# Rhizomatica/mercury

Measured on AMD Instinct MI355X. Metric: RX frames/s (mode 8, max 50 LDPC iters), higher is better.
Workload: dtype f64

## Files before the change

### include/mercury_gpu.h

```cpp
#ifndef MERCURY_GPU_H
#define MERCURY_GPU_H

#include <stddef.h>
#include <stdint.h>

#ifdef __cplusplus
extern "C" {
#endif

#define MGPU_OK 0
#define MGPU_ERR_ARG 1
#define MGPU_ERR_DEVICE 2
#define MGPU_ERR_TABLES 3
#define MGPU_ERR_UNSUPPORTED 4

#define MGPU_DEC_GBF 0
#define MGPU_DEC_SPA 1
#define MGPU_DEC_MINSUM 2
#define MGPU_DEC_SPA_FAST 3

#define MGPU_EST_ZF 0
#define MGPU_EST_LS 1

typedef struct mgpu_ctx mgpu_ctx;
// ... 6 lines not shown
         ? -1                                                                                                                     \
         : 1000 + (((MGPU_CFG_MOD_INDEX_(M) * 8 + MGPU_CFG_RATE_INDEX_(rate16)) * 8 + ((preamble_nsymb)-1)) * 2 + (estimator)))

typedef struct mgpu_config {
    int cfg;
    int max_iters;
    int decoder;
    int agc;
    int variance_source;
    int device;
    int max_batch;
    float minsum_alpha;
    int mfsk_ctrl_mode;
    int test_puncture_nBits;
} mgpu_config;

typedef struct mgpu_info {
    int cfg, M, bits_per_symbol, K, P, N;
    int Nsymb, Nc, Nfft, Ngi, Nofdm;
    int nData, nBits, nPilots, nVirtual, nReal;
    int bit_blk, tf_blk, preamble_nsymb;
    int estimator, amp_restore, ls_window;
    int Cwidth, Vwidth, E;
    int payload_bytes;
    int payload_stride;
    int frame_samples;
    int mfsk_M, mfsk_nStreams;
    int active_nsymb, active_nbits;
} mgpu_info;

typedef struct mgpu_frame_stats {
    int iterations_done;
    int crc;
    int all_zeros;
    int message_decoded;
    float variance;
    float snr_db;
} mgpu_frame_stats;

typedef struct mgpu_stage_taps {
    double* grid;
    double* H;
    double* eq;
    double* syms;
    float* llr_demod;
    float* llr_ldpc;
    double* variance;
    double* agc_gain;
    long long* cycles;
} mgpu_stage_taps;

int mgpu_create(const mgpu_config* cfg, mgpu_ctx** out);

typedef struct mgpu_explicit_params {
    float pilot_boost;
    int ls_window;
    int seeds_set;
    unsigned pilot_seed, scrambler_seed, preamble_seed;
    int Nc, Nfft, Dx;
    int Dy;
    int Nsymb;
} mgpu_explicit_params;
int mgpu_create_explicit(const mgpu_config* cfg, const mgpu_explicit_params* params, mgpu_ctx** out);
void mgpu_destroy(mgpu_ctx* ctx);
const char* mgpu_last_error(mgpu_ctx* ctx);
int mgpu_get_info(mgpu_ctx* ctx, mgpu_info* info);

void* mgpu_alloc_host(size_t bytes);
void mgpu_free_host(void* p);

typedef struct mgpu_device_props {
    int compute_units, clock_khz, memory_clock_khz, lds_bytes_per_cu, wavefront_size, numa_node;
    unsigned long long hbm_bytes;
    char name[64];
    char gcn_arch[32];
    char pci_bus_id[32];
} mgpu_device_props;
int mgpu_device_props_get(int device, mgpu_device_props* out);
void* mgpu_alloc_host_near(int device, size_t bytes);
int mgpu_host_numa_node_of_pci(const char* pci_bus_id);
int mgpu_host_numa_cpus(int node, int* cpus, int max);

int mgpu_rx_batch(mgpu_ctx* ctx, const double* baseband_c128, int F, uint8_t* payload,
                  mgpu_frame_stats* stats, float* llr_opt);
int mgpu_rx_batch_taps(mgpu_ctx* ctx, const double* baseband_c128, int F, uint8_t* payload,
                       mgpu_frame_stats* stats, const mgpu_stage_taps* taps);
int mgpu_ldpc_batch(mgpu_ctx* ctx, const float* llr, int F, uint8_t* bits, int* iters);
int mgpu_host_select_peak(const double* cand_vals, int ncand, int step, int size, int location_to_return, int nTrials_max, int* delay,
                          double* correlation);
int mgpu_host_fir_taps(int which, double carrier_hz, double* taps, int* ntaps);
int mgpu_host_preamble_carriers(int cfg, double* carriers_c128, int* n_symbols);
int mgpu_host_mode_info(int cfg, int mfsk_ctrl_mode, mgpu_info* info);
int mgpu_host_layout_stats(int cfg, double out[4]);

typedef struct mgpu_libm_report {
    long long evaluated[4], differed[4];
    double first_differing_argument[4];
    int differing;
    char libc_version[32];
} mgpu_libm_report;
int mgpu_host_libm_selfcheck(mgpu_libm_report* out );

int mgpu_ldpc_encode_batch(mgpu_ctx* ctx, const uint8_t* bits, int F, uint8_t* encoded);

int mgpu_rx_batch_dev(mgpu_ctx* ctx, const void* d_baseband_c128, int F, void* d_payload,
                      void* d_stats, void* d_llr_opt, void* stream);
int mgpu_frontend_dev(mgpu_ctx* ctx, const void* d_baseband_c128, int F, void* d_llr, void* d_variance_f,
                      void* stream);
int mgpu_ldpc_batch_dev(mgpu_ctx* ctx, const void* d_llr, int F, void* d_bits_opt, void* d_iters,
                        void* d_payload_opt, void* d_stats_opt, const void* d_variance_f_opt, void* stream);
void* mgpu_device_malloc(mgpu_ctx* ctx, size_t bytes);
void mgpu_device_free(mgpu_ctx* ctx, void* d_ptr);
void* mgpu_context_stream(mgpu_ctx* ctx);
int mgpu_synchronize(mgpu_ctx* ctx, void* stream_or_null);
int mgpu_copy_to_host(mgpu_ctx* ctx, void* dst, const void* d_src, size_t bytes, void* stream_or_null);
int mgpu_copy_to_device(mgpu_ctx* ctx, void* d_dst, const void* src, size_t bytes, void* stream_or_null);
int mgpu_txgen_dev(mgpu_ctx* ctx, uint64_t seed, uint64_t frame0, int F, double noise_amp, int channel,
                   void* d_baseband_c128, void* d_payload_opt, void* stream);

typedef struct mgpu_error_rate {
    double esn0_db;
    long long Frames_total, Error_frames_total, Bits_total, Error_bits_total;
    double BER, FER;
    double avg_iterations;
    long long crc_ok_frames;
} mgpu_error_rate;
int mgpu_baseband_test_esn0(mgpu_ctx* ctx, const double* esn0_db, int npoints, long long frames_per_point, uint64_t seed, uint64_t frame0,
                            int channel, mgpu_error_rate* out);

int mgpu_passband_to_baseband(mgpu_ctx* ctx, const double* passband , int W, int in_size,
                              const double* carrier_hz , int filter, const int* start , int count,
                              int decimation, double* out_c128 );
int mgpu_time_sync_preamble(mgpu_ctx* ctx, const double* baseband_interp_c128 , int W, int size, int step,
                            int location_to_return, int nTrials_max, int* delay , double* correlation );
int mgpu_freq_sync(mgpu_ctx* ctx, const double* baseband_c128 , int W, int stride, double* freq_offset_hz );
int mgpu_time_sync_mfsk(mgpu_ctx* ctx, const double* baseband_interp_c128 , int W, int size, int search_start_symb,
                        int* delay );
int mgpu_detect_ack_pattern(mgpu_ctx* ctx, const double* baseband_interp_c128 , int W, int size, int pattern,
                            double* metric , int* matched );
int mgpu_detect_ack_pattern_from_passband(mgpu_ctx* ctx, const double* passband , int W, int size, double carrier_hz,
                                          int pattern, double* metric , int* matched );
int mgpu_last_sync_kernel_ms(mgpu_ctx* ctx, float* ms);

int mgpu_enable_timing(mgpu_ctx* ctx, int on);
int mgpu_kernel_ms_avg(mgpu_ctx* ctx, float ms[2], int* n_launches);
int mgpu_decoder_hard_frames(mgpu_ctx* ctx, long long* frames);
int mgpu_host_path_last(mgpu_ctx* ctx, int* chunk_frames, int* n_chunks, float* fill_ms, float* drain_ms, float* total_ms);
int mgpu_last_kernel_ms(mgpu_ctx* ctx, float ms[2]);

int mgpu_debug_mfsk_sync(mgpu_ctx* ctx, const double* energy, int W, int nslots, int size, const int* search_start, int variant, int* delay);
int mgpu_debug_p2b_variant(int variant);
int mgpu_debug_span_energy(mgpu_ctx* ctx, const double* bb, int W, int size, const int* wv, const int* off, int n, int len, int variant, double* sum,
                           int* cnt);
int mgpu_debug_spa_math(mgpu_ctx* ctx, const double* in, int n, double* tanh_out, double* atanh_out);
int mgpu_debug_select_peak(mgpu_ctx* ctx, const double* cand_vals, int n, int ncand_max, const int* ncand, const int* size, const int* loc, int step,
                           int nTrials_max, int* delay, double* corr);

int mgpu_debug_occupancy(mgpu_ctx* ctx, int which);

int mgpu_debug_tsync_metric(mgpu_ctx* ctx, const double* baseband_interp, int W, int size, int step, int variant, const int* start, const int* sub_size,
                            double* vals);

int mgpu_debug_glibc_trig(mgpu_ctx* ctx, const double* in, int n, double* atan_out, double* sin_out, double* cos_out);

#ifdef __cplusplus
}
#endif
#endif
```

### mercury_amd/csrc/tables.cpp

```cpp
#include "tables.hpp"
#include "device_tables.h"

#include <algorithm>
#include <complex>
#include <cmath>
#include <cstring>
#include <future>
#include <map>
#include <memory>
#include <mutex>
#include <stdexcept>

namespace mgpu {

void GlibcRandom::reseed(unsigned seed) {
    if (seed == 0) seed = 1;
    st_[0] = static_cast<int32_t>(seed);
    int32_t word = st_[0];
    for (int i = 1; i < 31; ++i) {
        const long hi = word / 127773, lo = word % 127773;
        word = static_cast<int32_t>(16807 * lo - 2836 * hi);
        if (word < 0) word += 2147483647;
        st_[i] = word;
    }
    f_ = 3;
    r_ = 0;
    for (int k = 0; k < 310; ++k) (void)next();
}

int32_t GlibcRandom::next() {
    const uint32_t val = static_cast<uint32_t>(st_[f_]) + static_cast<uint32_t>(st_[r_]);
    st_[f_] = static_cast<int32_t>(val);
    if (++f_ >= 31) { f_ = 0; ++r_; }
    else if (++r_ >= 31) r_ = 0;
    return static_cast<int32_t>(val >> 1);
}

uint16_t crc16_modbus(const uint8_t* bytes, int n) {
    uint16_t crc = 0xffff;
    for (int j = 0; j < n; ++j) {
        crc ^= bytes[j];
        for (int i = 0; i < 8; ++i) crc = (crc & 1) ? static_cast<uint16_t>((crc >> 1) ^ 0xA001) : static_cast<uint16_t>(crc >> 1);
    }
    return crc;
}

namespace {

struct ModeRow { int M, rate16, preamble, estimator; };
constexpr ModeRow kModeTable[17] = {
    {2, 1, 4, 1},  {2, 2, 4, 1},  {2, 3, 4, 1},  {2, 4, 4, 1},  {2, 5, 4, 1},  {2, 6, 4, 1},
    {2, 8, 4, 1},  {4, 5, 4, 1},  {4, 6, 4, 1},  {4, 8, 4, 1},  {8, 6, 3, 1},  {8, 8, 3, 1},
    {4, 14, 3, 1}, {16, 8, 2, 1}, {8, 14, 2, 1}, {16, 14, 2, 0}, {32, 14, 1, 0},
};

constexpr int8_t kQam32[32][2] = {
    {-3, 5}, {-1, 5}, {-3, -5}, {-1, -5}, {-5, 3}, {-5, 1}, {-5, -3}, {-5, -1},
    {-1, 3}, {-1, 1}, {-1, -3}, {-1, -1}, {-3, 3}, {-3, 1}, {-3, -3}, {-3, -1},
    {3, 5},  {1, 5},  {3, -5},  {1, -5},  {5, 3},  {5, 1},  {5, -3},  {5, -1},
    {1, 3},  {1, 1},  {1, -3},  {1, -1},  {3, 3},  {3, 1},  {3, -3},  {3, -1}};

std::vector<Cplx> make_constellation(int M) {
    std::vector<Cplx> c(M);
    switch (M) {
        case 2: c = {{1, 0}, {-1, 0}}; break;
        case 4: c = {{-1, 1}, {-1, -1}, {1, 1}, {1, -1}}; break;
        case 8: {
            const double h = std::sqrt(2.0);
            const double p = (1 * h) / 2.0, n = (-1 * h) / 2.0;
            c = {{n, n}, {-1, 0}, {0, 1}, {n, p}, {0, -1}, {p, n}, {p, p}, {1, 0}};
            break;
        }
        case 16:
            for (int s = 0; s < 16; ++s)
                c[s] = {((s & 8) ? 1.0 : -1.0) * ((s & 4) ? 1.0 : 3.0), ((s & 2) ? -1.0 : 1.0) * ((s & 1) ? 1.0 : 3.0)};
            break;
        case 32:
            for (int s = 0; s < 32; ++s) c[s] = {double(kQam32[s][0]), double(kQam32[s][1])};
            break;
        default: throw std::runtime_error("unsupported constellation size");
    }
    float pnv = 0;
    for (const Cplx& z : c) pnv = static_cast<float>(static_cast<double>(pnv) + (z.re * z.re + z.im * z.im));
    const float mean = pnv / static_cast<float>(M);
    pnv = static_cast<float>(1.0 / std::sqrt(static_cast<double>(mean)));
    for (Cplx& z : c) { z.re *= static_cast<double>(pnv); z.im *= static_cast<double>(pnv); }
    return c;
}

std::vector<uint8_t> make_pilot_lattice(int Nsymb, int Nc, int Dy) {
    const int Dx = 1;
    const int S = Nc > Nsymb ? Nc : Nsymb;
    std::vector<uint8_t> v(size_t(S) * S, 0);
    for (int x = 0, y = 0; x < S && y < S; x += Dx, ++y) {
        for (int j = y; j < S; j += Dy) v[size_t(j) * S + x] = 1;
        for (int j = y; j >= 0; j -= Dy) v[size_t(j) * S + x] = 1;
    }
    int in_last = 0;
    for (int j = 0; j < Nsymb; ++j) in_last += v[size_t(j) * S + Nc - 1];
    if (in_last < 2)
        for (int j = 0; j < S; ++j) v[size_t(j) * S + Nc - 1] = v[size_t(j) * S];
    std::vector<uint8_t> t(size_t(Nsymb) * Nc);
    for (int j = 0; j < Nsymb; ++j)
        for (int i = 0; i < Nc; ++i) t[size_t(j) * Nc + i] = v[size_t(j) * S + i];
    return t;
}

static LdpcGraph load_graph_uncached(int K, const uint8_t* blob, size_t size) {
    auto rd32 = [&](size_t off) { uint32_t x; if (off + 4 > size) throw std::runtime_error("LDPC table blob truncated"); std::memcpy(&x, blob + off, 4); return x; };
    if (size < 12 || std::memcmp(blob, "MLDP", 4) != 0 || rd32(4) != 1) throw std::runtime_error("LDPC table blob: bad magic/version");
    const uint32_t nrates = rd32(8);
    size_t off = 12;
    for (uint32_t r = 0; r < nrates; ++r) {
        const uint32_t k = rd32(off), P = rd32(off + 4), N = rd32(off + 8), E = rd32(off + 12), cw = rd32(off + 16), vw = rd32(off + 20);
        off += 24;
        const size_t need = size_t(P) + 2 * size_t(E) + N + 2 * size_t(E);
        if (off + need > size) throw std::runtime_error("LDPC table blob truncated");
        if (int(k) != K) { off += need; continue; }
        LdpcGraph g;
        if (N != 1600) throw std::runtime_error("LDPC table blob: N must be 1600 (the decoders' LDS layout is fixed to it)");
        g.K = K; g.P = P; g.N = N; g.E = E; g.Cwidth = cw; g.Vwidth = vw;
        const uint8_t* cdeg = blob + off;
        const uint8_t* cflat = cdeg + P;
        const uint8_t* vdeg = cflat + 2 * size_t(E);
        const uint8_t* vflat = vdeg + N;
        g.cptr.resize(P + 1); g.cvar.resize(E); g.vptr.resize(N + 1); g.vedge.resize(E);
        uint32_t e = 0;
        for (uint32_t c = 0; c < P; ++c) {
            g.cptr[c] = e;
            for (uint32_t j = 0; j < cdeg[c]; ++j, ++e) {
                uint16_t v; std::memcpy(&v, cflat + 2 * size_t(e), 2);
                g.cvar[e] = v;
            }
        }
        g.cptr[P] = e;
        uint32_t s = 0;
        for (uint32_t v = 0; v < N; ++v) {
            g.vptr[v] = s;
            for (uint32_t j = 0; j < vdeg[v]; ++j, ++s) {
                uint16_t c; std::memcpy(&c, vflat + 2 * size_t(s), 2);
                uint32_t found = UINT32_MAX;
                for (uint32_t q = g.cptr[c]; q < g.cptr[c] + cdeg[c]; ++q)
                    if (g.cvar[q] == v) { found = q; break; }
                if (found == UINT32_MAX) throw std::runtime_error("LDPC table blob: C/V adjacency mismatch");
                g.vedge[s] = uint16_t(found);
            }
        }
        g.vptr[N] = s;
        if (s != E) throw std::runtime_error("LDPC table blob: edge count mismatch");
        std::vector<uint32_t> order(P);
        for (uint32_t c = 0; c < P; ++c) order[c] = c;
        std::stable_sort(order.begin(), order.end(), [&](uint32_t a, uint32_t b) { return cdeg[a] > cdeg[b]; });
        std::vector<int> fill;
        std::vector<std::vector<uint32_t>> members;
        for (uint32_t c : order) {
            const int d = cdeg[c];
            if (d > 64) throw std::runtime_error("check degree exceeds a wavefront");
            size_t b = 0;
            for (; b < fill.size(); ++b) if (fill[b] + d <= 64) break;
            if (b == fill.size()) { fill.push_back(0); members.emplace_back(); }
            fill[b] += d;
            members[b].push_back(c);
        }
        g.S = int(fill.size()) * 64;
        if (g.S >= 8192) throw std::runtime_error("padded edge count exceeds the 13-bit slot field");
        std::vector<uint32_t> slot_of_edge(E);
        for (size_t b = 0; b < members.size(); ++b) {
            uint32_t p = uint32_t(b) * 64;
            for (uint32_t c : members[b]) {
                const uint32_t d = cdeg[c];
                for (uint32_t j = 0; j < d; ++j, ++p) slot_of_edge[g.cptr[c] + j] = p;
            }
        }
        std::vector<uint32_t> vorder(N);
        for (uint32_t v = 0; v < N; ++v) vorder[v] = v;
        std::stable_sort(vorder.begin(), vorder.end(), [&](uint32_t a, uint32_t b) { return vdeg[a] > vdeg[b]; });
        g.vinfo.assign(size_t(N) * 8, 0u);
        for (uint32_t i = 0; i < N; ++i) {
            const uint32_t v = vorder[i], d = vdeg[v];
            if (d > uint32_t(kSpaMaxVarDegree)) throw std::runtime_error("variable degree exceeds the unrolled update (and the bound the fp64 decoder's hard-frame shortcut is proved with: device_tables.h kSpaMaxVarDegree)");
            if (i >= 1024 && d > 4) g.fp64_limit = "variable degrees exceed the fp64 decoder's register layout (rows from 1024 on: at most 4 edges)";
            g.vinfo[size_t(i) * 8] = v | (d << 11);
            for (uint32_t j = 0; j < d; ++j) {
                const uint32_t slot = slot_of_edge[g.vedge[g.vptr[v] + j]];
                g.vinfo[size_t(i) * 8 + 1 + j / 2] |= slot << (16 * (j & 1));
            }
        }
        {
            std::vector<std::vector<uint32_t>> by_kind(7);
            for (uint32_t c : order) {
                int k = 1;
                while ((1 << k) < int(cdeg[c])) ++k;
                by_kind[k].push_back(c);
            }
            std::vector<uint32_t> kinds;
            std::vector<std::vector<uint32_t>> bin_checks;
            for (int k = 6; k >= 1; --k) {
                const size_t per = size_t(64) >> k;
                for (size_t i = 0; i < by_kind[k].size(); i += per) {
                    kinds.push_back(uint32_t(k));
                    bin_checks.emplace_back(by_kind[k].begin() + i, by_kind[k].begin() + std::min(by_kind[k].size(), i + per));
                }
            }
            const size_t bins = kinds.size(), rounds = (bins + 7) / 8;
            g.Sg = int(bins) * 64;
            if (g.Sg >= 65536) throw std::runtime_error("grouped layout exceeds the 16-bit slot index of the variable records");
            if (rounds > 21) throw std::runtime_error("grouped layout exceeds the 21 rounds whose group sizes fit one 64-bit word per wavefront");
            g.gdesc.assign((rounds + 1) * 512, 0u);
            g.gkind.assign((rounds + 1) * 8, 0u);
            g.gkpack.assign(8, 0ull);
            std::vector<uint32_t> lane_of_edge(E), bin_of_edge(E), group_of_edge(E), gsize_of_edge(E);
            for (size_t b = 0; b < bins; ++b) {
                g.gkind[b] = kinds[b];
                g.gkpack[b & 7] |= uint64_t(kinds[b]) << (3 * (b >> 3));
                const uint32_t gsz = 1u << kinds[b];
                for (size_t q = 0; q < bin_checks[b].size(); ++q) {
                    const uint32_t c = bin_checks[b][q];
                    for (uint32_t j = 0; j < cdeg[c]; ++j) {
                        const uint32_t eo = g.cptr[c] + j;
                        lane_of_edge[eo] = uint32_t(q) * gsz + j;
                        bin_of_edge[eo] = uint32_t(b);
                        group_of_edge[eo] = c;
                        gsize_of_edge[eo] = gsz;
                    }
                }
            }
            std::vector<uint32_t> vorder_g = vorder, row_of(N);
            {
                std::vector<std::vector<uint32_t>> halves_of_var(N);
                for (uint32_t c = 0; c < P; ++c)
                    for (uint32_t j = 0; j < cdeg[c]; ++j) {
                        const uint32_t eo = g.cptr[c] + j, h = bin_of_edge[eo] * 2 + (lane_of_edge[eo] >= 32 ? 1u : 0u);
                        auto& hv = halves_of_var[g.cvar[eo]];
                        if (std::find(hv.begin(), hv.end(), h) == hv.end()) hv.push_back(h);
                    }
                std::vector<int> cnt(bins * 2 * 32, 0);
                auto bump = [&](uint32_t v, uint32_t bank, int d) { long long delta = 0; for (uint32_t h : halves_of_var[v]) { int& x = cnt[size_t(h) * 32 + bank]; delta += d > 0 ? 2 * x + 1 : 1 - 2 * x; x += d; } return delta; };
                for (uint32_t i = 0; i < N; ++i) bump(vorder_g[i], i & 31, +1);
                uint32_t lcg = 12345u;
                auto coin = [&] { lcg = lcg * 1664525u + 1013904223u; return (lcg >> 16) & 1u; };
                auto try_swap = [&](uint32_t ia, uint32_t ib) {
                    const uint32_t va = vorder_g[ia], vb = vorder_g[ib];
                    if ((ia & 31) == (ib & 31)) return false;
                    const long long d = bump(va, ia & 31, -1) + bump(vb, ib & 31, -1) + bump(va, ib & 31, +1) + bump(vb, ia & 31, +1);
                    if (d < 0 || (d == 0 && coin())) { std::swap(vorder_g[ia], vorder_g[ib]); return d < 0; }
                    bump(va, ib & 31, -1); bump(vb, ia & 31, -1); bump(va, ia & 31, +1); bump(vb, ib & 31, +1);
                    return false;
                };
                for (int sweep = 0, idle = 0; sweep < 200 && idle < 6; ++sweep) {
                    bool improved = false;
                    for (uint32_t ia = 0; ia < N; ++ia) {
                        const uint32_t lo = ia & ~31u, hi = std::min<uint32_t>(lo + 32, N);
                        for (uint32_t ib = ia + 1; ib < hi; ++ib) improved |= try_swap(ia, ib);
                        for (uint32_t ib = hi; ib < N && ib / 512 == ia / 512 && vdeg[vorder_g[ib]] == vdeg[vorder_g[ia]]; ++ib) improved |= try_swap(ia, ib);
                    }
                    idle = improved ? 0 : idle + 1;
                }
                for (uint32_t i = 0; i < N; ++i) row_of[vorder_g[i]] = i;
            }
            {
                std::vector<uint32_t> access_of_edge(E);
                for (uint32_t v = 0; v < N; ++v)
                    for (uint32_t j = 0; j < vdeg[v]; ++j) access_of_edge[g.vedge[g.vptr[v] + j]] = (row_of[v] / 32) * 9 + j;
                std::vector<int> cnt(size_t((N + 31) / 32) * 9 * 32, 0);
                auto at = [&](uint32_t e, uint32_t lane) -> int& { return cnt[size_t(access_of_edge[e]) * 32 + (lane & 31)]; };
                for (uint32_t e2 = 0; e2 < E; ++e2) ++at(e2, lane_of_edge[e2]);
                uint32_t lcg = 54321u;
                auto coin = [&] { lcg = lcg * 1664525u + 1013904223u; return (lcg >> 16) & 1u; };
                for (int sweep = 0, idle = 0; sweep < 200 && idle < 6; ++sweep) {
                    bool improved = false;
                    for (uint32_t c = 0; c < P; ++c) {
                        const uint32_t e0 = g.cptr[c], d = cdeg[c];
                        if (d == 0) continue;
                        const uint32_t gsz = gsize_of_edge[e0], gbase = lane_of_edge[e0] - (lane_of_edge[e0] % gsz);
                        std::vector<int> edge_at(gsz, -1);
                        for (uint32_t j = 0; j < d; ++j) edge_at[lane_of_edge[e0 + j] - gbase] = int(e0 + j);
                        for (uint32_t a = 0; a < gsz; ++a)
                            for (uint32_t b2 = a + 1; b2 < gsz; ++b2) {
                                if (((gbase + a) ^ (gbase + b2)) & 32) continue;
                                const int ea = edge_at[a], eb = edge_at[b2];
                                if (ea < 0 && eb < 0) continue;
                                long long dlt = 0;
                                auto mv = [&](int e2, uint32_t from, uint32_t to) { if (e2 < 0) return; int& x = at(uint32_t(e2), from); dlt += 1 - 2 * x; --x; int& y = at(uint32_t(e2), to); dlt += 2 * y + 1; ++y; };
                                mv(ea, gbase + a, gbase + b2); mv(eb, gbase + b2, gbase + a);
                                if (dlt < 0 || (dlt == 0 && coin())) {
                                    if (ea >= 0) lane_of_edge[ea] = gbase + b2;
                                    if (eb >= 0) lane_of_edge[eb] = gbase + a;
                                    std::swap(edge_at[a], edge_at[b2]);
                                    improved |= dlt < 0;
                                } else { mv(ea, gbase + b2, gbase + a); mv(eb, gbase + a, gbase + b2); }
                            }
                    }
                    for (size_t b = 0; b < bins; ++b) {
                        const uint32_t gsz = 1u << kinds[b];
                        if (gsz >= 32) continue;
                        const uint32_t per_half = 32 / gsz;
                        std::vector<std::vector<uint32_t>> members(64 / gsz);
                        for (uint32_t c : bin_checks[b])
                            for (uint32_t j = 0; j < cdeg[c]; ++j) members[lane_of_edge[g.cptr[c] + j] / gsz].push_back(g.cptr[c] + j);
                        for (uint32_t half = 0; half < 2; ++half)
                            for (uint32_t pa = 0; pa < per_half; ++pa)
                                for (uint32_t pb = pa + 1; pb < per_half; ++pb) {
                                    const uint32_t ga = half * per_half + pa, gb = half * per_half + pb;
                                    if (members[ga].empty() && members[gb].empty()) continue;
                                    const int shift = int(gb - ga) * int(gsz);
                                    long long dlt = 0;
                                    auto mvg = [&](const std::vector<uint32_t>& es, int sh) {
                                        for (uint32_t e2 : es) { int& x = at(e2, lane_of_edge[e2]); dlt += 1 - 2 * x; --x; }
                                        for (uint32_t e2 : es) { int& y = at(e2, uint32_t(int(lane_of_edge[e2]) + sh)); dlt += 2 * y + 1; ++y; }
                                    };
                                    mvg(members[ga], shift); mvg(members[gb], -shift);
                                    if (dlt < 0 || (dlt == 0 && coin())) {
                                        for (uint32_t e2 : members[ga]) lane_of_edge[e2] = uint32_t(int(lane_of_edge[e2]) + shift);
                                        for (uint32_t e2 : members[gb]) lane_of_edge[e2] = uint32_t(int(lane_of_edge[e2]) - shift);
                                        std::swap(members[ga], members[gb]);
                                        improved |= dlt < 0;
                                    } else {
// ... 276 lines not shown
        w[n] = pilot_boost * (1.0 / s);
    }
    return w;
}

ModeTables build_mode_tables(int cfg, int mfsk_ctrl_mode, const uint8_t* blob, size_t blob_size, const ExplicitParams& xp) {
    const bool robust = cfg >= 100 && cfg <= 102;
    ModeRow explicit_row = {0, 0, 0, 0};
    const bool is_explicit = explicit_mode_row(cfg, &explicit_row.M, &explicit_row.rate16, &explicit_row.preamble, &explicit_row.estimator);
    if (!robust && !is_explicit && (cfg < 0 || cfg > 16))
        throw std::runtime_error("cfg must be 0..16 (OFDM), 100..102 (ROBUST MFSK) or an MGPU_CFG_EXPLICIT id");
    const ModeRow robust_row = {200 , cfg == 102 ? 4 : 1, 4, 1};
    const ModeRow& row = robust ? robust_row : is_explicit ? explicit_row : kModeTable[cfg];
    ModeTables t;
    t.xp = xp;
    t.lsw = xp.ls_window % 2 == 0 ? xp.ls_window + 1 : xp.ls_window;
    if (!(xp.pilot_boost > 0.0f) || !(xp.pilot_boost < 1e6f)) throw std::runtime_error("pilot_boost must be a positive finite number");
    if (t.lsw < 1 || t.lsw > 21) throw std::runtime_error("LS window must be 1..21 cells wide (the front-end reads at most 7 pilots of a window row)");
    t.cfg = cfg;
    t.M = row.M;
    t.preamble = row.preamble;
    t.estimator = row.estimator;
    t.amp_restore = (row.M == 2 || row.M == 4 || row.M == 8) ? 1 : 0;
    t.K = static_cast<int>(static_cast<float>(t.N) * (row.rate16 / 16.0f));
    t.P = t.N - t.K;
    switch (row.M) {
        case 2: t.Nsymb = 48; t.bps = 1; break;
        case 4: t.Nsymb = 24; t.bps = 2; break;
        case 8: t.Nsymb = 16; t.bps = 3; break;
        case 16: t.Nsymb = 12; t.bps = 4; break;
        default: t.Nsymb = 9; t.bps = 5; break;
    }
    if (xp.Nsymb != 0 || xp.Dy != 3) {
        if (robust) throw std::runtime_error("explicit Nsymb / Dy: the MFSK modes take their frame length from the codeword (telecom_system.cc:1812-1816) and carry no pilots");
        if (xp.Nsymb < 0 || xp.Nsymb > 255 || xp.Dy < 1 || xp.Dy > 255) throw std::runtime_error("explicit Nsymb / Dy out of range");
        if (xp.Nsymb > 0) t.Nsymb = xp.Nsymb;
    }
    if (robust) {
        t.mfsk_M = cfg == 100 ? 32 : 16;
        t.mfsk_nstreams = cfg == 100 ? 1 : 2;
        t.mfsk_nbits = cfg == 100 ? 5 : 4;
        t.mfsk_hop = t.mfsk_M == 32 ? 13 : 7;
        const int global_offset = (t.Nc - t.mfsk_nstreams * t.mfsk_M) / 2;
        for (int k = 0; k < t.mfsk_nstreams; ++k) t.mfsk_off[k] = global_offset + k * t.mfsk_M;
        t.mfsk_amp = std::sqrt(double(t.Nc) / t.mfsk_nstreams);
        t.bps = t.mfsk_nbits * t.mfsk_nstreams;
        t.Nsymb = t.N / t.bps;
        t.ctrl_nbits = cfg == 100 ? 1200 : cfg == 101 ? 1400 : 0;
        t.ctrl_nsymb = t.ctrl_nbits / t.bps;
    }
    const int G = t.Nsymb * t.Nc;
    t.cell_type = robust ? std::vector<uint8_t>(G, 0) : make_pilot_lattice(t.Nsymb, t.Nc, xp.Dy);
    t.pilot_boost = static_cast<double>(xp.pilot_boost);
    t.pilot_val.assign(G, 0.0);
    if (!robust) {
        GlibcRandom rng(xp.pilot_seed);
        int last = 0;
        for (int c = 0; c < G; ++c) {
            if (!t.cell_type[c]) continue;
            const int pv = (rng.next() % 2) ^ last;
            t.pilot_val[c] = double(2 * pv - 1) * t.pilot_boost;
            last = pv;
            ++t.nPilots;
        }
    }
    t.nData = robust ? t.Nsymb : G - t.nPilots;
    t.nBits = t.nData * t.bps;
    t.nVirtual = t.N - t.nBits;
    t.nReal = t.nBits - t.P;
    if (t.nVirtual < 0 || t.nVirtual > t.K || t.nReal < 24)
        throw std::runtime_error("frame geometry: the data cells hold " + std::to_string(t.nBits) + " bits - more than a codeword, fewer than its parity + a payload byte, or more virtual bits than information bits");
    t.bit_blk = t.nBits / 10;
    t.tf_blk = t.nData / 10;
    t.payload_bytes = (t.nReal - 16) / 8;
    t.payload_stride = (t.nReal + 7) / 8;
    {
        const bool on = mfsk_ctrl_mode && robust && t.ctrl_nbits > 0 && t.ctrl_nbits < t.nBits;
        t.active_nsymb = (on && t.ctrl_nsymb > 0) ? t.ctrl_nsymb : t.Nsymb;
        t.active_nbits = (on && t.ctrl_nbits > 0) ? t.ctrl_nbits : t.nBits;
    }
    t.frame_samples = t.active_nsymb * t.Nofdm;
    if (!robust) t.constellation = make_constellation(t.M);
    {
        GlibcRandom rng(xp.scrambler_seed);
        t.scrambler.resize(t.N);
        for (int i = 0; i < t.N; ++i) t.scrambler[i] = uint8_t(rng.next() % 2);
    }
    t.twiddle.resize(128);
    for (int k = 0; k < 128; ++k) {
        const double angle = -2.0 * M_PI * k / 256;
        t.twiddle[k] = {std::cos(angle), std::sin(angle)};
    }
    std::vector<uint16_t> data_cell;
    for (int c = 0; c < G && int(data_cell.size()) < t.nData; ++c) if (!t.cell_type[c]) data_cell.push_back(uint16_t(c));
    auto deint_src = [](int n, int bs) {
        std::vector<int> src(n);
        const int nb = n / bs;
        for (int i = 0; i < nb; ++i) for (int j = 0; j < bs; ++j) src[i * bs + j] = j * nb + i;
        for (int i = nb * bs; i < n; ++i) src[i] = i;
        return src;
    };
    const std::vector<int> tf = deint_src(t.nData, t.tf_blk);
    t.sym_src.resize(t.nData);
    t.tf_inv.resize(t.nData);
    for (int k = 0; k < t.nData; ++k) { t.sym_src[k] = data_cell[tf[k]]; t.tf_inv[tf[k]] = uint16_t(k); }
    t.data_cell = data_cell;
    const std::vector<int> bd = deint_src(t.nBits, t.bit_blk);
    t.llr_src.resize(t.N);
    for (int p = 0; p < t.N; ++p) {
        int d;
        if (p < t.nReal) d = p;
        else if (p < t.nReal + t.nVirtual) d = p - t.nReal;
        else d = p - t.nVirtual;
        t.llr_src[p] = uint16_t(bd[d]);
    }
    if (robust) {
        if (t.nVirtual != 0) throw std::runtime_error("MFSK mode with virtual bits");
        t.llr_dst.assign(t.nBits, 0);
        for (int p = 0; p < t.N; ++p) t.llr_dst[t.llr_src[p]] = uint16_t(p);
    }
    t.ls_weight = ls_weight_table(t.pilot_boost, t.lsw * t.lsw);
    t.bit_il.resize(t.nBits);
    for (int i = 0; i < t.nBits; ++i) t.bit_il[bd[i]] = uint16_t(i);
    t.sym_cell.resize(t.nData);
    for (int k = 0; k < t.nData; ++k) t.sym_cell[k] = t.sym_src[k];
    t.preamble_carriers.assign(size_t(t.preamble) * t.Nc, Cplx{0.0, 0.0});
    if (t.mfsk_M > 0) {
        static constexpr int kTones32[4] = {4, 20, 12, 28}, kTones16[4] = {2, 10, 6, 14};
        const int* tones = t.mfsk_M == 32 ? kTones32 : kTones16;
        for (int s = 0; s < t.preamble; ++s)
            for (int st = 0; st < t.mfsk_nstreams; ++st) t.preamble_carriers[size_t(s) * t.Nc + t.mfsk_off[st] + tones[s % 4]] = Cplx{t.mfsk_amp, 0.0};
    } else {
        GlibcRandom rng(xp.preamble_seed);
        const double s2 = std::sqrt(2.0);
        for (int i = 0; i < t.preamble; ++i)
            for (int j = 0; j < t.Nc; ++j) {
                const int bin = j < t.Nc / 2 ? j + t.Nfft - t.Nc / 2 : j - t.Nc / 2 + 1;
                if (bin % 2 == 1) continue;
                const int im = 2 * (rng.next() % 2) - 1;
                const int re = 2 * (rng.next() % 2) - 1;
                t.preamble_carriers[size_t(i) * t.Nc + j] = Cplx{double(re) / s2, double(im) / s2};
            }
    }
    {
        const double bandwidth = 48000.0 * 50.0 / 256 / 4, fs = 48000.0;
        t.fir_time_sync = design_lpf_hamming(3000.0, 0.9 * bandwidth / 2, fs);
        t.fir_data = design_lpf_hamming(3000.0, 1.0 * bandwidth / 2, fs);
    }
    t.graph = load_graph(t.K, blob, blob_size);
    if (t.graph.P != t.P) throw std::runtime_error("LDPC graph does not match the mode");
    return t;
}

}
```

### mercury_amd/physical_layer.py

```python
import ctypes as C
import os

import numpy as np

HERE = os.path.dirname(os.path.abspath(__file__))
LIB_PATH = os.environ.get("MERCURY_GPU_LIB") or os.path.join(HERE, "libmercury_gpu.so")

DEC_GBF, DEC_SPA, DEC_MINSUM, DEC_SPA_FAST = 0, 1, 2, 3
EST_ZF, EST_LS = 0, 1


class Config(C.Structure):
    _fields_ = [("cfg", C.c_int), ("max_iters", C.c_int), ("decoder", C.c_int), ("agc", C.c_int),
                ("variance_source", C.c_int), ("device", C.c_int), ("max_batch", C.c_int),
                ("minsum_alpha", C.c_float), ("mfsk_ctrl_mode", C.c_int), ("test_puncture_nBits", C.c_int)]


INFO_FIELDS = ("cfg M bits_per_symbol K P N Nsymb Nc Nfft Ngi Nofdm nData nBits nPilots nVirtual nReal "
               "bit_blk tf_blk preamble_nsymb estimator amp_restore ls_window Cwidth Vwidth E "
               "payload_bytes payload_stride frame_samples mfsk_M mfsk_nStreams active_nsymb active_nbits").split()


class ExplicitParams(C.Structure):
    _fields_ = [("pilot_boost", C.c_float), ("ls_window", C.c_int), ("seeds_set", C.c_int), ("pilot_seed", C.c_uint),
                ("scrambler_seed", C.c_uint), ("preamble_seed", C.c_uint), ("Nc", C.c_int), ("Nfft", C.c_int), ("Dx", C.c_int), ("Dy", C.c_int), ("Nsymb", C.c_int)]


class Info(C.Structure):
    _fields_ = [(n, C.c_int) for n in INFO_FIELDS]


class Taps(C.Structure):
    _fields_ = [(n, C.c_void_p) for n in "grid H eq syms llr_demod llr_ldpc variance agc_gain cycles".split()]


class ReceiveConfig(C.Structure):
    _fields_ = [("carrier_hz", C.c_double), ("time_sync_trials_max", C.c_int), ("use_last_good_time_sync", C.c_int),
                ("use_last_good_freq_offset", C.c_int), ("coarse_freq_sync_enabled", C.c_int)]


class TransmitConfig(C.Structure):
    _fields_ = [("carrier_hz", C.c_double), ("carrier_amplitude", C.c_double), ("output_power_watt", C.c_double),
                ("preamble_papr_cut", C.c_double), ("data_papr_cut", C.c_double), ("start_sample", C.c_uint64),
                ("message_location", C.c_int), ("phase_continuous", C.c_int)]


FIRST_MESSAGE, MIDDLE_MESSAGE, FLUSH_MESSAGE = 0, 1, 2
SINGLE_MESSAGE, NO_FILTER_MESSAGE, BATCH_MESSAGE = 3, 4, 16

LINK_STATE_DTYPE = np.dtype([("delay_of_last_decoded_message", "<i4"), ("freq_offset_of_last_decoded_message", "<f8"),
                             ("mfsk_search_start", "<i4"), ("fixed_delay_plus_one", "<i4")], align=True)
RECEIVE_STATS_DTYPE = np.dtype([("iterations_done", "<i4"), ("crc", "<i4"), ("all_zeros", "<i4"), ("message_decoded", "<i4"),
                                ("snr_db", "<f8"), ("delay", "<i4"), ("sync_trials", "<i4"), ("freq_offset", "<f8"),
                                ("coarse_metric", "<f8"), ("frame_overflow_symbols", "<i4"), ("mean_H", "<f8"),
                                ("signal_strength_dbm", "<f8")], align=True)

STATS_DTYPE = np.dtype([("iterations_done", "<i4"), ("crc", "<i4"), ("all_zeros", "<i4"),
                        ("message_decoded", "<i4"), ("variance", "<f4"), ("snr_db", "<f4")])

_lib = None


def load_library():
    global _lib
    if _lib is None:
        if not os.path.exists(LIB_PATH):
            raise RuntimeError(
                "%s is missing: run `python -c 'import __graft_entry__ as g; g.build()'` "
                "(the Mercury RX path has no CPU fallback)" % LIB_PATH)
        try:
            import torch
        except Exception:
            pass
        lib = C.CDLL(LIB_PATH)
        lib.mgpu_last_error.restype = C.c_char_p
        lib.mgpu_last_error.argtypes = [C.c_void_p]
        lib.mgpu_create.argtypes = [C.POINTER(Config), C.POINTER(C.c_void_p)]
        lib.mgpu_txgen_dev.argtypes = [C.c_void_p, C.c_uint64, C.c_uint64, C.c_int, C.c_double, C.c_int,
                                       C.c_void_p, C.c_void_p, C.c_void_p]
        lib.mgpu_rx_batch_dev.argtypes = [C.c_void_p, C.c_void_p, C.c_int, C.c_void_p, C.c_void_p, C.c_void_p, C.c_void_p]
        lib.mgpu_frontend_dev.argtypes = [C.c_void_p, C.c_void_p, C.c_int, C.c_void_p, C.c_void_p, C.c_void_p]
        lib.mgpu_ldpc_batch_dev.argtypes = [C.c_void_p, C.c_void_p, C.c_int, C.c_void_p, C.c_void_p, C.c_void_p,
                                            C.c_void_p, C.c_void_p, C.c_void_p]
        lib.mgpu_destroy.argtypes = [C.c_void_p]
        _hf_argtypes(lib)
        _div_argtypes(lib)
        _lib = lib
    return _lib


EXPORTED_SYMBOLS = [
    "mgpu_alloc_host", "mgpu_free_host", "mgpu_create", "mgpu_destroy", "mgpu_last_error", "mgpu_get_info", "mgpu_rx_batch", "mgpu_rx_batch_taps",
    "mgpu_host_libm_selfcheck", "mgpu_host_select_peak", "mgpu_host_fir_taps", "mgpu_host_preamble_carriers", "mgpu_host_mode_info", "mgpu_host_layout_stats",
    "mgpu_device_props_get", "mgpu_alloc_host_near", "mgpu_host_numa_node_of_pci", "mgpu_host_numa_cpus", "mgpu_pool_device_numa_node",
    "mgpu_ldpc_batch", "mgpu_ldpc_encode_batch", "mgpu_rx_batch_dev", "mgpu_frontend_dev", "mgpu_ldpc_batch_dev", "mgpu_txgen_dev",
    "mgpu_host_path_last", "mgpu_device_malloc", "mgpu_device_free", "mgpu_context_stream", "mgpu_synchronize", "mgpu_copy_to_host", "mgpu_copy_to_device",
    "mgpu_pool_rx_batch_dev", "mgpu_pool_ldpc_batch_dev", "mgpu_pool_txgen_dev",
    "mgpu_last_kernel_ms", "mgpu_kernel_ms_avg", "mgpu_decoder_hard_frames", "mgpu_enable_timing", "mgpu_debug_spa_math", "mgpu_debug_glibc_trig", "mgpu_debug_tsync_metric", "mgpu_debug_occupancy", "mgpu_debug_select_peak", "mgpu_debug_span_energy", "mgpu_debug_p2b_variant", "mgpu_debug_mfsk_sync", "mgpu_baseband_test_esn0", "mgpu_passband_test_esn0", "mgpu_passband_to_baseband", "mgpu_time_sync_preamble", "mgpu_freq_sync", "mgpu_last_sync_kernel_ms",
    "mgpu_time_sync_mfsk", "mgpu_detect_ack_pattern", "mgpu_detect_ack_pattern_from_passband",
    "mgpu_receive_buffer_nsymb", "mgpu_receive_byte_batch", "mgpu_receive_byte_batch_samples", "mgpu_measure_signal_only",
    "mgpu_host_pre_equalization_channel", "mgpu_context_pre_equalization_channel", "mgpu_set_pre_equalization_channel", "mgpu_transmit_bit_batch", "mgpu_transmit_frame_samples", "mgpu_transmit_byte_batch", "mgpu_transmit_byte_batch_dev", "mgpu_transmit_buffer", "mgpu_symbol_mod", "mgpu_generate_ack_pattern_passband",
    "mgpu_symbol_demod", "mgpu_automatic_gain_control", "mgpu_channel_estimator", "mgpu_restore_channel_amplitude", "mgpu_channel_equalizer",
    "mgpu_measure_variance", "mgpu_deframer", "mgpu_deinterleaver_c128", "mgpu_deinterleaver_f32", "mgpu_psk_demod",
    "mgpu_bit_energy_dispersal", "mgpu_bit_to_byte", "mgpu_crc16_modbus_rtu",
    "mgpu_shm_create", "mgpu_shm_connect", "mgpu_shm_close", "mgpu_shm_destroy", "mgpu_shm_used", "mgpu_shm_free", "mgpu_shm_capacity",
    "mgpu_shm_clear", "mgpu_shm_write", "mgpu_shm_read", "mgpu_shm_read_all", "mgpu_shm_publish_decoded",
    "mgpu_create_explicit", "mgpu_pool_create", "mgpu_pool_destroy", "mgpu_pool_size", "mgpu_pool_context", "mgpu_pool_last_error", "mgpu_pool_last_counters",
    "mgpu_pool_shard", "mgpu_pool_rx_batch", "mgpu_pool_ldpc_batch", "mgpu_pool_receive_byte_batch",
]


ESTIMATOR_SYMBOLS = ["mgpu_set_estimator_ladder", "mgpu_get_estimator_ladder", "mgpu_estimator_rungs_last", "mgpu_estimator_ladder_counters",
                     "mgpu_host_ls_estimate", "mgpu_set_estimator_ladder_ex", "mgpu_get_estimator_ladder_ex", "mgpu_host_wiener_estimate",
                     "mgpu_host_wiener_tables"]
LADDER_MAX = 4
RUNG_LS, RUNG_WIENER = 0, 1
WIENER_DESIGN_DEFAULT = dict(tau_min_us=-333.33, tau_max_us=2333.33, doppler_hz=0.5, snr_db=0.0)


class LsWindow(C.Structure):
    _fields_ = [("width", C.c_int), ("height", C.c_int)]


class WienerDesign(C.Structure):
    _fields_ = [("tau_min_us", C.c_double), ("tau_max_us", C.c_double), ("doppler_hz", C.c_double), ("snr_db", C.c_double)]


class EstimatorRung(C.Structure):
    _fields_ = [("kind", C.c_int), ("window", LsWindow), ("design", WienerDesign)]


def _wiener_design(design):
    d = dict(WIENER_DESIGN_DEFAULT)
    for k, v in (design or {}).items():
        if k not in d:
            raise MgpuError("a Wiener design has %s, not %r" % (sorted(d), k))
        d[k] = float(v)
    return WienerDesign(d["tau_min_us"], d["tau_max_us"], d["doppler_hz"], d["snr_db"])


def parse_ladder(text):
    if not text:
        return []
    rungs = []
    for item in text.split(","):
        item = item.strip().lower()
        if rungs and isinstance(rungs[-1][1], dict) and "=" in item and "x" not in item.split("=")[0] and not item.startswith(("wiener", "bank")):
            key, value = item.split("=", 1)
        elif item.startswith("bank"):
            if not item.startswith("bank:") or "=" not in item:
                raise MgpuError("a bank rung is 'bank:tau=MIN/MAX|MIN/MAX|...,fd=HZ,snr=DB,rho=R|R', not %r" % item)
            rungs.append(("bank", {}))
            key, value = item[len("bank:"):].split("=", 1)
        elif item.startswith("wiener"):
            rungs.append(("wiener", {}))
            if item == "wiener":
                continue
            if not item.startswith("wiener:") or "=" not in item:
                raise MgpuError("a Wiener rung is 'wiener' or 'wiener:tau=MIN/MAX,fd=HZ,snr=DB', not %r" % item)
            key, value = item[len("wiener:"):].split("=", 1)
        else:
            rungs.append(tuple(int(v) for v in item.split("x")))
            continue
        d = rungs[-1][1]
        if rungs[-1][0] == "bank" and key in ("tau", "rho"):
            if key == "tau":
                d["tau"] = [tuple(float(v) for v in iv.split("/")) for iv in value.split("|")]
                if any(len(iv) != 2 for iv in d["tau"]):
                    raise MgpuError("a bank's intervals are MIN/MAX, separated by '|', not %r" % value)
            else:
                d["rho"] = [float(v) for v in value.split("|")]
        elif key == "tau":
            lo, hi = value.split("/")
            d["tau_min_us"], d["tau_max_us"] = float(lo), float(hi)
        elif key in ("fd", "snr"):
            d["doppler_hz" if key == "fd" else "snr_db"] = float(value)
        else:
            raise MgpuError("a Wiener rung's fields are tau, fd and snr, not %r" % key)
    for kind, d in [r for r in rungs if isinstance(r[1], dict) and r[0] == "bank"]:
        if not d.get("tau"):
            raise MgpuError("a bank rung needs tau=MIN/MAX|MIN/MAX|...")
        if "rho" in d and len(d["rho"]) != len(d["tau"]) - 1:
            raise MgpuError("a bank of %d designs takes %d rho values" % (len(d["tau"]), len(d["tau"]) - 1))
    return rungs


def _is_wiener(rung):
    return rung == "wiener" or (isinstance(rung, (tuple, list)) and len(rung) == 2 and rung[0] == "wiener")


WIENER_BANK_SYMBOLS = ["mgpu_set_wiener_bank", "mgpu_get_wiener_bank", "mgpu_get_wiener_choice", "mgpu_host_wiener_select",
                       "mgpu_host_wiener_bank_thresholds"]
WIENER_BANK_MAX = 4


class WienerBankEntry(C.Structure):
    _fields_ = [("design", WienerDesign), ("rho_min", C.c_double)]


def _is_bank(rung):
    return isinstance(rung, (tuple, list)) and len(rung) == 2 and rung[0] == "bank"


def bank_entries(spec):
    common = {k: spec[k] for k in ("doppler_hz", "snr_db") if k in spec}
    rho = list(spec.get("rho", [])) + [None] * len(spec["tau"])
    return [(dict(common, tau_min_us=lo, tau_max_us=hi), rho[i]) for i, (lo, hi) in enumerate(spec["tau"])]


def _bank_array(entries):
    entries = list(entries or [])
    arr = (WienerBankEntry * max(len(entries), 1))()
    for i, e in enumerate(entries):
        design, rho = e if isinstance(e, (tuple, list)) else (e, None)
        arr[i] = WienerBankEntry(_wiener_design(design), float("nan") if rho is None else float(rho))
    return arr, len(entries)


def host_wiener_select(cfg, grid, entries, explicit=None):
    lib = load_library()
    lib.mgpu_host_wiener_select.argtypes = [C.c_int, C.c_void_p, C.c_void_p, C.c_int, C.c_size_t, C.c_void_p, C.c_void_p, C.c_void_p, C.c_void_p, C.c_void_p]
    g = np.ascontiguousarray(grid, np.complex128).ravel()
    xp = _explicit_struct(explicit)
    arr, n = _bank_array(entries)
    design, n1, n2, corr = C.c_int(), C.c_int(), C.c_int(), np.zeros(4, np.float64)
    rc = lib.mgpu_host_wiener_select(int(cfg), C.byref(xp) if xp is not None else None, arr, n, C.sizeof(WienerBankEntry), _ptr(g), C.byref(design),
                                     _ptr(corr), C.byref(n1), C.byref(n2))
    if rc != 0:
        raise MgpuError("mgpu_host_wiener_select failed (%d)" % rc, rc)
    return dict(design=design.value, corr=corr, n1=n1.value, n2=n2.value)


def host_wiener_bank_thresholds(cfg, entries, explicit=None):
    lib = load_library()
    lib.mgpu_host_wiener_bank_thresholds.argtypes = [C.c_int, C.c_void_p, C.c_void_p, C.c_int, C.c_size_t, C.c_void_p, C.c_void_p]
    xp = _explicit_struct(explicit)
    arr, n = _bank_array(entries)
    rho, s = np.zeros(max(n - 1, 1), np.float64), C.c_int()
    rc = lib.mgpu_host_wiener_bank_thresholds(int(cfg), C.byref(xp) if xp is not None else None, arr, n, C.sizeof(WienerBankEntry), _ptr(rho), C.byref(s))
    if rc != 0:
        raise MgpuError("mgpu_host_wiener_bank_thresholds failed (%d)" % rc, rc)
    return rho[: max(n - 1, 0)], s.value


def wiener_sounding(corr, n1, n2, s):
    corr = np.asarray(corr, np.float64)
    r1, r2 = corr[..., 0] + 1j * corr[..., 1], corr[..., 2] + 1j * corr[..., 3]
    with np.errstate(divide="ignore", invalid="ignore"):
        rho = (np.abs(r2) / n2) / (np.abs(r1) / n1)
    return rho, -np.angle(r1) * 256.0 / (2.0 * np.pi * s) / 0.012

# ... 1506 lines not shown
```

Baseline: 729,900.

## Pack LDPC check nodes into fewer wavefront bins with dense DP packing

Replaces the first-fit-decreasing packing of check nodes into 64-lane edge bins with an exact subset-sum style packer that searches for the smallest bin count whose walk-group cost is no worse than FFD. Fewer bins shrink the padded edge slot count S, reducing wasted lanes and memory traffic per LDPC iteration. It also adds a debug export for inspecting the bin layout. Table construction gets more expensive, but that runs once at graph load and does not touch the decode kernel code.

```diff
diff --git a/include/mercury_gpu.h b/include/mercury_gpu.h
--- a/include/mercury_gpu.h
+++ b/include/mercury_gpu.h
@@ -182,6 +182,7 @@
 int mgpu_debug_p2b_variant(int variant);
 int mgpu_debug_span_energy(mgpu_ctx* ctx, const double* bb, int W, int size, const int* wv, const int* off, int n, int len, int variant, double* sum,
                            int* cnt);
+int mgpu_debug_spa_bins(int K, int dims[6], uint32_t* sadr, uint64_t* bhead, uint64_t* bmask);
 int mgpu_debug_spa_math(mgpu_ctx* ctx, const double* in, int n, double* tanh_out, double* atanh_out);
 int mgpu_debug_select_peak(mgpu_ctx* ctx, const double* cand_vals, int n, int ncand_max, const int* ncand, const int* size, const int* loc, int step,
                            int nTrials_max, int* delay, double* corr);
diff --git a/mercury_amd/csrc/tables.cpp b/mercury_amd/csrc/tables.cpp
--- a/mercury_amd/csrc/tables.cpp
+++ b/mercury_amd/csrc/tables.cpp
@@ -104,6 +104,110 @@
     for (int j = 0; j < Nsymb; ++j)
         for (int i = 0; i < Nc; ++i) t[size_t(j) * Nc + i] = v[size_t(j) * S + i];
     return t;
+}
+
+typedef std::vector<std::vector<uint32_t>> SpaBins;
+
+static SpaBins pack_ffd(const uint8_t* cdeg, const std::vector<uint32_t>& order) {
+    std::vector<int> fill;
+    SpaBins members;
+    for (uint32_t c : order) {
+        const int d = cdeg[c];
+        size_t b = 0;
+        for (; b < fill.size(); ++b) if (fill[b] + d <= 64) break;
+        if (b == fill.size()) { fill.push_back(0); members.emplace_back(); }
+        fill[b] += d;
+        members[b].push_back(c);
+    }
+    return members;
+}
+
+static long spa_walk_groups(const uint8_t* cdeg, const SpaBins& bins, int q) {
+    long w = 0;
+    for (const auto& bin : bins) {
+        int mx = 0;
+        for (uint32_t c : bin) mx = std::max(mx, int(cdeg[c]));
+        w += (mx + q - 1) / q;
+    }
+    return w;
+}
+
+static bool pack_dense(const uint8_t* cdeg, const std::vector<uint32_t>& order, size_t nb, int q, SpaBins& out) {
+    int cnt[65] = {0};
+    size_t next[65];
+    long edges = 0, left = 0;
+    for (size_t i = order.size(); i-- > 0;) {
+        const int d = cdeg[order[i]];
+        if (d == 0) return false;
+        ++cnt[d]; next[d] = i; edges += d; ++left;
+    }
+    long slack = long(nb) * 64 - edges;
+    if (slack < 0) return false;
+    out.clear();
+    bool below[65][65], in_class[66][65];
+    auto take = [&](int d, int k) { for (; k > 0; --k) { out.back().push_back(order[next[d]++]); --cnt[d]; --left; } };
+    while (left > 0) {
+        if (out.size() == nb) return false;
+        int m = 64;
+        while (!cnt[m]) --m;
+        out.emplace_back();
+        take(m, 1);
+        const int room = 64 - m;
+        for (int s = 0; s <= room; ++s) below[0][s] = s == 0;
+        for (int d = 1; d <= m; ++d)
+            for (int s = 0; s <= room; ++s) {
+                below[d][s] = false;
+                for (int k = 0; k <= cnt[d] && k * d <= s && !below[d][s]; ++k) below[d][s] = below[d - 1][s - k * d];
+            }
+        int t = -1;
+        for (int c = (m + q - 1) / q; c >= 1 && t != 0; --c) {
+            const int lo = q * (c - 1), hi = std::min(q * c, m), nd = hi - lo, lim = t < 0 ? room : t;
+            for (int s = 0; s <= lim; ++s) in_class[0][s] = s == 0;
+            for (int i = 1; i <= nd; ++i)
+                for (int s = 0; s <= lim; ++s) {
+                    const int d = lo + i;
+                    in_class[i][s] = false;
+                    for (int k = 0; k <= cnt[d] && k * d <= s && !in_class[i][s]; ++k) in_class[i][s] = in_class[i - 1][s - k * d];
+                }
+            int sc = -1;
+            if (t < 0) {
+                for (int tt = room; tt >= 0 && room - tt <= slack; --tt)
+                    for (int s = tt; s > sc; --s)
+                        if (in_class[nd][s] && below[lo][tt - s]) { sc = s; t = tt; break; }
+                if (sc < 0) return false;
+                slack -= room - t;
+            } else {
+                for (int s = t; s >= 0 && sc < 0; --s)
+                    if (in_class[nd][s] && below[lo][t - s]) sc = s;
+            }
+            t -= sc;
+            for (int i = nd; i >= 1; --i) {
+                const int d = lo + i;
+                int k = std::min(cnt[d], sc / d);
+                while (!in_class[i - 1][sc - k * d]) --k;
+                take(d, k);
+                sc -= k * d;
+            }
+        }
+    }
+    return true;
+}
+
+static SpaBins pack_spa_bins(const uint8_t* cdeg, const std::vector<uint32_t>& order) {
+    long edges = 0;
+    int maxdeg = 0;
+    for (uint32_t c : order) {
+        if (cdeg[c] > 64) throw std::runtime_error("check degree exceeds a wavefront");
+        edges += cdeg[c];
+        maxdeg = std::max(maxdeg, int(cdeg[c]));
+    }
+    SpaBins ffd = pack_ffd(cdeg, order);
+    const long w2 = spa_walk_groups(cdeg, ffd, 2), w4 = spa_walk_groups(cdeg, ffd, 4);
+    for (size_t nb = size_t(std::max(1l, (edges + 63) / 64)); nb < ffd.size(); ++nb) {
+        SpaBins dense;
+        if (pack_dense(cdeg, order, nb, maxdeg > 16 ? 4 : 2, dense) && spa_walk_groups(cdeg, dense, 2) <= w2 && spa_walk_groups(cdeg, dense, 4) <= w4) return dense;
+    }
+    return ffd;
 }
 
 static LdpcGraph load_graph_uncached(int K, const uint8_t* blob, size_t size) {
@@ -151,18 +255,8 @@
         std::vector<uint32_t> order(P);
         for (uint32_t c = 0; c < P; ++c) order[c] = c;
         std::stable_sort(order.begin(), order.end(), [&](uint32_t a, uint32_t b) { return cdeg[a] > cdeg[b]; });
-        std::vector<int> fill;
-        std::vector<std::vector<uint32_t>> members;
-        for (uint32_t c : order) {
-            const int d = cdeg[c];
-            if (d > 64) throw std::runtime_error("check degree exceeds a wavefront");
-            size_t b = 0;
-            for (; b < fill.size(); ++b) if (fill[b] + d <= 64) break;
-            if (b == fill.size()) { fill.push_back(0); members.emplace_back(); }
-            fill[b] += d;
-            members[b].push_back(c);
-        }
-        g.S = int(fill.size()) * 64;
+        const std::vector<std::vector<uint32_t>> members = pack_spa_bins(cdeg, order);
+        g.S = int(members.size()) * 64;
         if (g.S >= 8192) throw std::runtime_error("padded edge count exceeds the 13-bit slot field");
         std::vector<uint32_t> slot_of_edge(E);
         for (size_t b = 0; b < members.size(); ++b) {
@@ -745,4 +839,18 @@
     return t;
 }
 
-}
+extern "C" const unsigned char mgpu_ldpc_blob[];
+extern "C" const unsigned long mgpu_ldpc_blob_size;
+extern "C" int mgpu_debug_spa_bins(int K, int dims[6], uint32_t* sadr, uint64_t* bhead, uint64_t* bmask) {
+    if (!dims) return 1;
+    try {
+        const LdpcGraph g = load_graph_uncached(K, mgpu_ldpc_blob, mgpu_ldpc_blob_size);
+        dims[0] = g.S; dims[1] = g.DM; dims[2] = int(g.bmask.size() / (16 * size_t(g.DM))); dims[3] = g.N; dims[4] = g.E; dims[5] = g.P;
+        if (sadr) std::memcpy(sadr, g.sadr.data(), g.sadr.size() * sizeof(uint32_t));
+        if (bhead) std::memcpy(bhead, g.bhead.data(), g.bhead.size() * sizeof(uint64_t));
+        if (bmask) std::memcpy(bmask, g.bmask.data(), g.bmask.size() * sizeof(uint64_t));
+        return 0;
+    } catch (const std::exception&) { return 1; }
+}
+
+}
diff --git a/mercury_amd/physical_layer.py b/mercury_amd/physical_layer.py
--- a/mercury_amd/physical_layer.py
+++ b/mercury_amd/physical_layer.py
@@ -96,7 +96,7 @@
     "mgpu_ldpc_batch", "mgpu_ldpc_encode_batch", "mgpu_rx_batch_dev", "mgpu_frontend_dev", "mgpu_ldpc_batch_dev", "mgpu_txgen_dev",
     "mgpu_host_path_last", "mgpu_device_malloc", "mgpu_device_free", "mgpu_context_stream", "mgpu_synchronize", "mgpu_copy_to_host", "mgpu_copy_to_device",
     "mgpu_pool_rx_batch_dev", "mgpu_pool_ldpc_batch_dev", "mgpu_pool_txgen_dev",
-    "mgpu_last_kernel_ms", "mgpu_kernel_ms_avg", "mgpu_decoder_hard_frames", "mgpu_enable_timing", "mgpu_debug_spa_math", "mgpu_debug_glibc_trig", "mgpu_debug_tsync_metric", "mgpu_debug_occupancy", "mgpu_debug_select_peak", "mgpu_debug_span_energy", "mgpu_debug_p2b_variant", "mgpu_debug_mfsk_sync", "mgpu_baseband_test_esn0", "mgpu_passband_test_esn0", "mgpu_passband_to_baseband", "mgpu_time_sync_preamble", "mgpu_freq_sync", "mgpu_last_sync_kernel_ms",
+    "mgpu_last_kernel_ms", "mgpu_kernel_ms_avg", "mgpu_decoder_hard_frames", "mgpu_enable_timing", "mgpu_debug_spa_math", "mgpu_debug_spa_bins", "mgpu_debug_glibc_trig", "mgpu_debug_tsync_metric", "mgpu_debug_occupancy", "mgpu_debug_select_peak", "mgpu_debug_span_energy", "mgpu_debug_p2b_variant", "mgpu_debug_mfsk_sync", "mgpu_baseband_test_esn0", "mgpu_passband_test_esn0", "mgpu_passband_to_baseband", "mgpu_time_sync_preamble", "mgpu_freq_sync", "mgpu_last_sync_kernel_ms",
     "mgpu_time_sync_mfsk", "mgpu_detect_ack_pattern", "mgpu_detect_ack_pattern_from_passband",
     "mgpu_receive_buffer_nsymb", "mgpu_receive_byte_batch", "mgpu_receive_byte_batch_samples", "mgpu_measure_signal_only",
     "mgpu_host_pre_equalization_channel", "mgpu_context_pre_equalization_channel", "mgpu_set_pre_equalization_channel", "mgpu_transmit_bit_batch", "mgpu_transmit_frame_samples", "mgpu_transmit_byte_batch", "mgpu_transmit_byte_batch_dev", "mgpu_transmit_buffer", "mgpu_symbol_mod", "mgpu_generate_ack_pattern_passband",
```

New measurement: 739,500, median of 6. +1.3%, better.
